# IceTTTb/NopeSAC

Measured on AMD Instinct MI355X. Metric: image-pairs/sec (480x640, K=32 hyp), higher is better.
Workload: dtype bf16; 1 GPU; configs/inference_mp3d.yaml, 32 synthetic 480x640 pairs/GPU/step, ResNet-50 + pyramids in bfloat16, head GEMMs bf16 operands with f32 accumulate / residual stream / LayerNorm / softmax, K=32 matched planes forced (m mean 32.0), nq=50; pairs_per_gpu=32, global_batch=32, K=32, parallelism=pair-sharded dp1, rccl_ranks=1, batches_in_flight_per_gpu=4, hip_graph=False, steps_per_all_gather=8, routing_entries_loaded=45, routing_entries_measured_now=0, nonfinite_outputs=0

## Files before the change

nopesac_amd/csrc/postselect.hip:

```cpp
#include "common.h"

namespace nps {

__host__ __device__ inline int work_words(int nq) { return 9 * nq + 8; }

__global__ __launch_bounds__(64) void ps_classify_kernel(const float* __restrict__ logits, int nq, float score_thr,
                                                         int* __restrict__ work) {
    const int b = blockIdx.x, lane = threadIdx.x;
    int* wk = work + (long long)b * work_words(nq);
    const float* lg = logits + (long long)b * nq * 2;
    int any = 0;
    float best_p0 = -1.f;
    int best_q = 0x7fffffff;
    for (int q = lane; q < nq; q += 64) {
        const float l0 = lg[2 * q], l1 = lg[2 * q + 1];
        const float mx = fmaxf(l0, l1);
        const float e0 = expf(l0 - mx), e1 = expf(l1 - mx);
        const float p0 = e0 / (e0 + e1), p1 = e1 / (e0 + e1);
        const int label = p1 > p0 ? 1 : 0;
        const float score = label ? p1 : p0;
        const int valid = (label == 0) && (score > score_thr);
        wk[q] = valid;
        wk[nq + q] = __float_as_int(score);
        any |= valid;
        if (p0 > best_p0) { best_p0 = p0; best_q = q; }
    }
    any = __any(any);
    if (!any) {
        for (int o = 32; o > 0; o >>= 1) {
            const float op = __shfl_xor(best_p0, o, 64);
            const int oq = __shfl_xor(best_q, o, 64);
            if (op > best_p0 || (op == best_p0 && oq < best_q)) { best_p0 = op; best_q = oq; }
        }
        if (lane == 0) {
            wk[best_q] = 1;
            wk[nq + best_q] = __float_as_int(best_p0);
        }
    }
    if (lane == 0) wk[9 * nq] = any ? 0 : 1;
}

constexpr int PS_TW = 64;
__host__ __device__ inline int ps_pad4(int nq) { return (nq + 3) & ~3; }
__host__ __device__ inline int ps_head_words(int nq) { return ((9 * nq + 3) & ~3) + 2 * ps_pad4(nq) + 4; }

__device__ __forceinline__ int mask_lane_sum(unsigned long long m) {
    return __popcll(m & 0xAAAAAAAAAAAAAAAAull) + 2 * __popcll(m & 0xCCCCCCCCCCCCCCCCull) + 4 * __popcll(m & 0xF0F0F0F0F0F0F0F0ull) +
           8 * __popcll(m & 0xFF00FF00FF00FF00ull) + 16 * __popcll(m & 0xFFFF0000FFFF0000ull) + 32 * __popcll(m & 0xFFFFFFFF00000000ull);
}

__device__ __forceinline__ int ps_writelane(int value, int lane_index, int old) {
    int saved_m0;
    asm volatile("s_mov_b32 %1, m0\n\ts_nop 4\n\ts_mov_b32 m0, %3\n\ts_nop 1\n\tv_writelane_b32 %0, %2, m0\n\ts_mov_b32 m0, %1"
                 : "+v"(old), "=&s"(saved_m0) : "s"(value), "s"(lane_index));
    return old;
}

template <int ROWS, bool X4>
__global__ __launch_bounds__(256) void ps_pixels_kernel(const float* __restrict__ prob, int nq, int h, int w, int H,
                                                        int W, float mask_thr, int src_rows, int src_cols,
                                                        int* __restrict__ work, uint8_t* __restrict__ winner, int planar, int th) {
    extern __shared__ __attribute__((aligned(16))) int sh[];
    const int nqp = ps_pad4(nq), acc_words = (9 * nq + 3) & ~3;
    int* vq = sh + acc_words;
    float* vs = reinterpret_cast<float*>(vq + nqp);
    int* nvp = vq + 2 * nqp;
    float* tile = reinterpret_cast<float*>(sh + ps_head_words(nq));
    const int b = blockIdx.z, lane = threadIdx.x & 63;
    const int wave = __builtin_amdgcn_readfirstlane(threadIdx.x >> 6);
    int* wk = work + (long long)b * work_words(nq);
    const float sch = (float)h / (float)H, scw = (float)w / (float)W;
    const int X0 = blockIdx.x * PS_TW, Y0 = blockIdx.y * th;
    const int ry0 = min((int)fmaxf(sch * (Y0 + 0.5f) - 0.5f, 0.f), h - 1);
    const int cx0 = min((int)fmaxf(scw * (X0 + 0.5f) - 0.5f, 0.f), w - 1);
    const int nrows = min(src_rows, h - ry0), ncols = min(src_cols, w - cx0);
    for (int i = threadIdx.x; i < 9 * nq; i += 256) sh[i] = 0;
    if (wave == 0) {
        int off = 0;
        for (int base = 0; base < nq; base += 64) {
            const int q = base + lane, qc = q < nq ? q : nq - 1;
            const int vl = wk[qc], sl = wk[nq + qc];
            const int v = q < nq ? vl : 0;
            const unsigned long long m = __ballot(v != 0);
            if (v) {
                const int pos = off + __popcll(m & ((1ull << lane) - 1ull));
                vq[pos] = q;
                vs[pos] = __int_as_float(sl);
            }
            off += __popcll(m);
        }
        if (lane == 0) *nvp = off;
    }
    __syncthreads();
    const int nv = *nvp, kp = ps_pad4(nv), nk4 = kp >> 2;
    if (nv == 0) return;
    if (threadIdx.x < kp - nv) { vq[nv + threadIdx.x] = vq[nv - 1]; vs[nv + threadIdx.x] = -1.f; }
    __syncthreads();
    {
        const unsigned inv = ((1u << 20) + nk4 - 1) / nk4;
        const int items = nrows * ncols * nk4;
        const long long plane = (long long)h * w;
        for (int it0 = threadIdx.x; it0 < items; it0 += 4 * 256) {
            float4 v[4];
            int dst[4];
#pragma unroll
            for (int u = 0; u < 4; ++u) {
                const int it = it0 + u * 256 < items ? it0 + u * 256 : items - 1;
                const int rc = (int)(((unsigned)it * inv) >> 20), k4 = it - rc * nk4;
                const int r = rc / ncols, c = rc - r * ncols;
                const int4 q4 = *reinterpret_cast<const int4*>(vq + 4 * k4);
                const long long pix = (long long)(ry0 + r) * w + cx0 + c;
                if (planar) {
                    const float* pb = prob + (long long)b * nq * plane + pix;
                    v[u] = make_float4(pb[q4.x * plane], pb[q4.y * plane], pb[q4.z * plane], pb[q4.w * plane]);
                } else {
                    const float* pb = prob + ((long long)b * plane + pix) * nq;
                    v[u] = make_float4(pb[q4.x], pb[q4.y], pb[q4.z], pb[q4.w]);
                }
                dst[u] = (r * src_cols + c) * kp + 4 * k4;
            }
#pragma unroll
            for (int u = 0; u < 4; ++u)
                if (it0 + u * 256 < items) *reinterpret_cast<float4*>(tile + dst[u]) = v[u];
        }
    }
    __syncthreads();
    const int X = X0 + lane;
    const float sx = fmaxf(scw * (X + 0.5f) - 0.5f, 0.f);
    const int x0 = min((int)sx, w - 1), x1 = min(x0 + 1, w - 1);
    const float lx = sx - x0, hx = 1.f - lx;
    const int c0 = min(max(x0 - cx0, 0), ncols - 1), c1 = min(max(x1 - cx0, 0), ncols - 1);
    float hy[ROWS], ly[ROWS], best[ROWS];
    int win[ROWS];
    const float *p00[ROWS], *p01[ROWS], *p10[ROWS], *p11[ROWS];
    unsigned long long inm[ROWS];
    bool in[ROWS];
#pragma unroll
    for (int r = 0; r < ROWS; ++r) {
        const int Y = X4 ? Y0 + wave * 4 + r : Y0 + r * 4 + wave;
        in[r] = X < W && Y < H;
        inm[r] = __ballot(in[r]);
        const float sy = fmaxf(sch * (Y + 0.5f) - 0.5f, 0.f);
        const int y0 = min((int)sy, h - 1), y1 = min(y0 + 1, h - 1);
        ly[r] = sy - y0; hy[r] = 1.f - ly[r];
        const int r0 = min(max(y0 - ry0, 0), nrows - 1), r1 = min(max(y1 - ry0, 0), nrows - 1);
        p00[r] = tile + (r0 * src_cols + c0) * kp; p01[r] = tile + (r0 * src_cols + c1) * kp;
        p10[r] = tile + (r1 * src_cols + c0) * kp; p11[r] = tile + (r1 * src_cols + c1) * kp;
        best[r] = -INFINITY; win[r] = -1;
    }
    int cnt_lo = 0, cnt_hi = 0;
    for (int k4 = 0; k4 < nk4; ++k4) {
        const int4 q4 = *reinterpret_cast<const int4*>(vq + 4 * k4);
        const float4 s4 = *reinterpret_cast<const float4*>(vs + 4 * k4);
        const int qv[4] = {q4.x, q4.y, q4.z, q4.w};
        const float sv[4] = {s4.x, s4.y, s4.z, s4.w};
        int np[4] = {0, 0, 0, 0};
        if constexpr (X4) {
            static_assert(!X4 || ROWS == 4, "X4 needs four rows per wave");
            float T[3][4];
#pragma unroll
            for (int sr = 0; sr < 3; ++sr) {
                const float* pa = sr == 0 ? p00[0] : (sr == 1 ? p00[2] : p10[2]);
                const float* pb = sr == 0 ? p01[0] : (sr == 1 ? p01[2] : p11[2]);
                const float4 a = *reinterpret_cast<const float4*>(pa + 4 * k4), bq = *reinterpret_cast<const float4*>(pb + 4 * k4);
                const float av[4] = {a.x, a.y, a.z, a.w}, bv[4] = {bq.x, bq.y, bq.z, bq.w};
#pragma unroll
                for (int e = 0; e < 4; ++e) T[sr][e] = hx * av[e] + lx * bv[e];
            }
#pragma unroll
            for (int r = 0; r < ROWS; ++r) {
#pragma unroll
                for (int e = 0; e < 4; ++e) {
                    const float p = hy[r] * T[r >> 1][e] + ly[r] * T[(r >> 1) + 1][e];
                    const float wgt = sv[e] * p;
                    if (wgt > best[r]) { best[r] = wgt; win[r] = qv[e]; }
                    np[e] += __popcll(__builtin_amdgcn_ballot_w64(p >= mask_thr) & inm[r]);
                }
            }
        } else
#pragma unroll
        for (int r = 0; r < ROWS; ++r) {
            const float4 a = *reinterpret_cast<const float4*>(p00[r] + 4 * k4), bq = *reinterpret_cast<const float4*>(p01[r] + 4 * k4);
            const float4 c = *reinterpret_cast<const float4*>(p10[r] + 4 * k4), d = *reinterpret_cast<const float4*>(p11[r] + 4 * k4);
            const float av[4] = {a.x, a.y, a.z, a.w}, bv[4] = {bq.x, bq.y, bq.z, bq.w}, cv[4] = {c.x, c.y, c.z, c.w}, dv[4] = {d.x, d.y, d.z, d.w};
#pragma unroll
            for (int e = 0; e < 4; ++e) {
                const float p = hy[r] * (hx * av[e] + lx * bv[e]) + ly[r] * (hx * cv[e] + lx * dv[e]);
                const float wgt = sv[e] * p;
                if (wgt > best[r]) { best[r] = wgt; win[r] = qv[e]; }
                np[e] += __popcll(__builtin_amdgcn_ballot_w64(p >= mask_thr) & inm[r]);
            }
        }
#pragma unroll
        for (int e = 0; e < 4; ++e) {
            const int k = 4 * k4 + e;
            if (k4 < 16) cnt_lo = ps_writelane(np[e], k, cnt_lo);
            else cnt_hi = ps_writelane(np[e], k - 64, cnt_hi);
        }
    }
#pragma unroll
    for (int r = 0; r < ROWS; ++r) {
        const int Y = X4 ? Y0 + wave * 4 + r : Y0 + r * 4 + wave;
        const bool ok = in[r] && win[r] >= 0;
        const bool pass = ok && best[r] > mask_thr;
        if (ok) winner[((long long)b * H + Y) * W + X] = (uint8_t)(win[r] | (pass ? 0x80 : 0));
        unsigned long long rem = __ballot(ok);
        while (rem) {
            const int w0 = __builtin_amdgcn_readlane(win[r], __ffsll((long long)rem) - 1);
            const unsigned long long m = __ballot(ok && win[r] == w0), mp = __ballot(pass && win[r] == w0);
            if (lane == 0) {
                const int cnt = __popcll(m), cp = __popcll(mp);
                atomicAdd(&sh[6 * nq + w0], cnt); atomicAdd(&sh[7 * nq + w0], X0 * cnt + mask_lane_sum(m)); atomicAdd(&sh[8 * nq + w0], Y * cnt);
                if (cp) { atomicAdd(&sh[3 * nq + w0], cp); atomicAdd(&sh[4 * nq + w0], X0 * cp + mask_lane_sum(mp)); atomicAdd(&sh[5 * nq + w0], Y * cp); }
            }
            rem &= ~m;
        }
    }
    if (lane < nv && cnt_lo) atomicAdd(&sh[2 * nq + vq[lane]], cnt_lo);
    if (lane + 64 < nv && cnt_hi) atomicAdd(&sh[2 * nq + vq[lane + 64]], cnt_hi);
    __syncthreads();
    for (int i = 2 * nq + threadIdx.x; i < 9 * nq; i += 256)
        if (sh[i]) atomicAdd(&wk[i], sh[i]);
}

__global__ __launch_bounds__(64) void ps_finalize_kernel(const float* __restrict__ params, const float* __restrict__ feat,
                                                         int nq, int D, int H, int W, float overlap_thr,
                                                         const int* __restrict__ work, int* __restrict__ n_kept,
                                                         int* __restrict__ kept_idx, float* __restrict__ planes,
                                                         float* __restrict__ feats, float* __restrict__ scores,
                                                         int* __restrict__ areas, float* __restrict__ centers,
                                                         uint8_t* __restrict__ winner, int* __restrict__ flags) {
    const int b = blockIdx.x, lane = threadIdx.x;
    const int* wk = work + (long long)b * work_words(nq);
    __shared__ int s_keep[128];
    __shared__ int s_n, s_fallback;
    const int zero_flag = wk[9 * nq];
    if (lane == 0) {
        int n = 0, fb = 0;
        double max_overlap = 0.0;
        int max_overlap_q = -1, first_valid = -1;
        for (int q = 0; q < nq; ++q) {
            if (!wk[q]) continue;
            if (first_valid < 0) first_valid = q;
            const int area = wk[3 * nq + q], orig = wk[2 * nq + q];
            if (!zero_flag) {
                if (area < 1 || orig < 1) continue;
                const double overlap = (double)area / (double)orig;
                if (overlap > max_overlap) { max_overlap = overlap; max_overlap_q = q; }
                if (overlap < (double)overlap_thr) continue;
            }
            s_keep[n++] = q;
        }
        if (n == 0) {
            s_keep[0] = max_overlap_q >= 0 ? max_overlap_q : first_valid;
            n = 1;
            fb = 1;
        }
        s_n = n;
        s_fallback = fb;
        n_kept[b] = n;
        flags[b] = (zero_flag ? 1 : 0) | (fb ? 2 : 0);
    }
    __syncthreads();
    const int n = s_n, fb = s_fallback;
    for (int i = lane; i < nq; i += 64) {
        const long long o = (long long)b * nq + i;
        if (i < n) {
            const int q = s_keep[i];
            int area, sxi, syi;
            double cx, cy;
            if (fb) {
                area = wk[6 * nq + q]; sxi = wk[7 * nq + q]; syi = wk[8 * nq + q];
                cx = ((double)sxi / W) / (double)area;
                cy = ((double)syi / H) / (double)area;
            } else {
                area = wk[3 * nq + q]; sxi = wk[4 * nq + q]; syi = wk[5 * nq + q];
                if (zero_flag && area == 0) {
                    area = 1; sxi = 0; syi = 0;
                    winner[(long long)b * H * W] = (uint8_t)(q | 0x80);
                }
                cx = ((double)sxi / W) / ((double)area + 1e-10);
                cy = ((double)syi / H) / ((double)area + 1e-10);
            }
            kept_idx[o] = q;
            areas[o] = area;
            scores[o] = __int_as_float(wk[nq + q]);
            centers[2 * o] = (float)cx;
            centers[2 * o + 1] = (float)cy;
            for (int d = 0; d < 3; ++d) planes[3 * o + d] = params[((long long)b * nq + q) * 3 + d];
        } else {
            kept_idx[o] = -1; areas[o] = 0; scores[o] = 0.f; centers[2 * o] = 0.f; centers[2 * o + 1] = 0.f;
            for (int d = 0; d < 3; ++d) planes[3 * o + d] = 0.f;
        }
    }
    for (int i = 0; i < nq; ++i) {
        const int q = i < n ? s_keep[i] : -1;
        for (int d = lane; d < D; d += 64)
            feats[((long long)b * nq + i) * D + d] = q >= 0 ? feat[((long long)b * nq + q) * D + d] : 0.f;
    }
}

}

extern "C" int nopesac_postselect_planes(const float* cls_logits, const float* mask_prob, const float* params,
                                         const float* query_feat, int B, int nq, int D, int h, int w, int H, int W,
                                         float score_thr, float mask_thr, float overlap_thr, int32_t* n_kept,
                                         int32_t* kept_idx, float* planes, float* feats, float* scores,
                                         int32_t* areas, float* centers, uint8_t* winner, int32_t* flags,
                                         int32_t* work, void* stream) {
    return nopesac_postselect_planes_ex(cls_logits, mask_prob, params, query_feat, B, nq, D, h, w, H, W, score_thr, mask_thr, overlap_thr,
                                        n_kept, kept_idx, planes, feats, scores, areas, centers, winner, flags, work, 0, stream);
}

extern "C" int nopesac_postselect_planes_ex(const float* cls_logits, const float* mask_prob, const float* params,
                                            const float* query_feat, int B, int nq, int D, int h, int w, int H, int W,
                                            float score_thr, float mask_thr, float overlap_thr, int32_t* n_kept,
                                            int32_t* kept_idx, float* planes, float* feats, float* scores,
                                            int32_t* areas, float* centers, uint8_t* winner, int32_t* flags,
                                            int32_t* work, int prob_planar, void* stream) {
    using namespace nps;
    NPS_CHECK_ARG(prob_planar == 0 || prob_planar == 1, "postselect: prob_planar must be 0 ([B,h,w,nq]) or 1 ([B,nq,h,w])");
    NPS_CHECK_ARG(cls_logits && mask_prob && params && query_feat && n_kept && kept_idx && planes && feats && scores &&
                      areas && centers && winner && flags && work, "postselect: null pointer");
    NPS_CHECK_ARG(B > 0 && nq > 0 && nq <= 128 && D > 0 && h > 0 && w > 0 && H > 0 && W > 0, "postselect: bad dims (nq<=128)");
    hipStream_t st = (hipStream_t)stream;
    hipError_t e = hipMemsetAsync(work, 0, (size_t)B * work_words(nq) * sizeof(int), st);
    if (e != hipSuccess) { set_error("postselect: memset failed: %s", hipGetErrorString(e)); return (int)e; }
    hipLaunchKernelGGL(ps_classify_kernel, dim3(B), dim3(64), 0, st, cls_logits, nq, score_thr, work);
    int th = 16, src_rows = 0;
    if (const char* e = getenv("NOPESAC_PS_TH")) { const int v = atoi(e); th = v >= 32 ? 32 : (v >= 16 ? 16 : (v >= 8 ? 8 : 4)); }
    const int src_cols = (int)(((long long)PS_TW * w + W - 1) / W) + 2;
    size_t lds = 0;
    for (;; th >>= 1) {
        src_rows = (int)(((long long)th * h + H - 1) / H) + 2;
        lds = (size_t)ps_head_words(nq) * sizeof(int) + (size_t)src_rows * src_cols * ps_pad4(nq) * sizeof(float);
        if (lds <= 64 * 1024 || th == 4) break;
    }
    NPS_CHECK_ARG(lds <= 64 * 1024, "postselect: up-sampling ratio too small for the LDS tile (%zu bytes)", lds);
    dim3 grid((W + PS_TW - 1) / PS_TW, (H + th - 1) / th, B);
    auto launch_pixels = [&](auto kern) {
        hipLaunchKernelGGL(kern, grid, dim3(256), lds, st, mask_prob, nq, h, w, H, W, mask_thr, src_rows, src_cols, work, winner,
                           prob_planar, th);
    };
    static const bool x4_off = getenv("NOPESAC_PS_X4") && atoi(getenv("NOPESAC_PS_X4")) == 0;
    if (th == 4) launch_pixels(ps_pixels_kernel<1, false>);
    else if (th == 8) launch_pixels(ps_pixels_kernel<2, false>);
    else if (th == 16 && H == 4 * h && !x4_off) launch_pixels(ps_pixels_kernel<4, true>);
    else if (th == 16) launch_pixels(ps_pixels_kernel<4, false>);
    else launch_pixels(ps_pixels_kernel<8, false>);
    hipLaunchKernelGGL(ps_finalize_kernel, dim3(B), dim3(64), 0, st, params, query_feat, nq, D, H, W, overlap_thr, work,
                       n_kept, kept_idx, planes, feats, scores, areas, centers, winner, flags);
    NPS_LAUNCH_RET();
}
```

Baseline: 4071 pairs/s.

## Prune plane candidates per tile using min/max mask-probability bounds

After loading the source tile into LDS, each block computes the per-query min and max probability over the tile with LDS atomics. It then derives a lower bound on the winning score. Queries that can never win and whose threshold outcome is uniform are dropped from the per-pixel argmax loop, and their counts are credited in bulk. This cuts the inner-loop work when few planes compete in a tile, at the cost of an extra reduction pass and barrier, and relies on the epsilon margins being safe for exactness.

```diff
diff --git a/nopesac_amd/csrc/postselect.hip b/nopesac_amd/csrc/postselect.hip
--- a/nopesac_amd/csrc/postselect.hip
+++ b/nopesac_amd/csrc/postselect.hip
@@ -41,6 +41,9 @@
 }
 
 constexpr int PS_TW = 64;
+constexpr float PS_EPS = 9.5367431640625e-07f;
+constexpr float PS_TINY = 7.888609052210118e-31f;
+constexpr unsigned PS_ONE_BITS = 0x3f800000u;
 __host__ __device__ inline int ps_pad4(int nq) { return (nq + 3) & ~3; }
 __host__ __device__ inline int ps_head_words(int nq) { return ((9 * nq + 3) & ~3) + 2 * ps_pad4(nq) + 4; }
 
@@ -59,7 +62,8 @@
 template <int ROWS, bool X4>
 __global__ __launch_bounds__(256) void ps_pixels_kernel(const float* __restrict__ prob, int nq, int h, int w, int H,
                                                         int W, float mask_thr, int src_rows, int src_cols,
-                                                        int* __restrict__ work, uint8_t* __restrict__ winner, int planar, int th) {
+                                                        int* __restrict__ work, uint8_t* __restrict__ winner, int planar, int th,
+                                                        int prune) {
     extern __shared__ __attribute__((aligned(16))) int sh[];
     const int nqp = ps_pad4(nq), acc_words = (9 * nq + 3) & ~3;
     int* vq = sh + acc_words;
@@ -92,9 +96,12 @@
         if (lane == 0) *nvp = off;
     }
     __syncthreads();
-    const int nv = *nvp, kp = ps_pad4(nv), nk4 = kp >> 2;
+    const int nv = __builtin_amdgcn_readfirstlane(*nvp), kp = ps_pad4(nv), nk4 = kp >> 2;
     if (nv == 0) return;
     if (threadIdx.x < kp - nv) { vq[nv + threadIdx.x] = vq[nv - 1]; vs[nv + threadIdx.x] = -1.f; }
+    unsigned* mnb = reinterpret_cast<unsigned*>(sh);
+    unsigned* mxb = mnb + nq;
+    if (prune && threadIdx.x < nv) mnb[threadIdx.x] = 0xffffffffu;
     __syncthreads();
     {
         const unsigned inv = ((1u << 20) + nk4 - 1) / nk4;
@@ -125,6 +132,20 @@
         }
     }
     __syncthreads();
+    if (prune) {
+        const int k = threadIdx.x % kp, g = threadIdx.x / kp, ng = 256 / kp, npos = nrows * ncols;
+        if (g < ng && k < nv) {
+            const unsigned inv = ((1u << 20) + ncols - 1) / ncols;
+            unsigned lo = 0xffffffffu, hi = 0u;
+            for (int p = g; p < npos; p += ng) {
+                const int r = (int)(((unsigned)p * inv) >> 20), c = p - r * ncols;
+                const unsigned bits = __float_as_uint(tile[(r * src_cols + c) * kp + k]);
+                lo = min(lo, bits); hi = max(hi, bits);
+            }
+            atomicMin(&mnb[k], lo); atomicMax(&mxb[k], hi);
+        }
+        __syncthreads();
+    }
     const int X = X0 + lane;
     const float sx = fmaxf(scw * (X + 0.5f) - 0.5f, 0.f);
     const int x0 = min((int)sx, w - 1), x1 = min(x0 + 1, w - 1);
@@ -149,7 +170,37 @@
         best[r] = -INFINITY; win[r] = -1;
     }
     int cnt_lo = 0, cnt_hi = 0;
+    unsigned long long cand_lo = nv >= 64 ? ~0ull : (1ull << nv) - 1ull, cand_hi = nv <= 64 ? 0ull : (nv >= 128 ? ~0ull : (1ull << (nv - 64)) - 1ull);
+    if (prune) {
+        int tot = 0;
+#pragma unroll
+        for (int r = 0; r < ROWS; ++r) tot += __popcll(inm[r]);
+        const bool thr_ok = mask_thr >= PS_TINY;
+        bool good[2], real[2];
+        float mn[2], mx[2], sc[2];
+        float lb = 0.f;
+#pragma unroll
+        for (int half = 0; half < 2; ++half) {
+            const int k = lane + 64 * half, kc = min(k, nv - 1);
+            real[half] = k < nv;
+            const unsigned hi = mxb[kc];
+            good[half] = real[half] && hi <= PS_ONE_BITS;
+            mn[half] = __uint_as_float(mnb[kc]); mx[half] = __uint_as_float(hi); sc[half] = vs[kc];
+            if (good[half]) lb = fmaxf(lb, sc[half] * (mn[half] * (1.f - PS_EPS)));
+        }
+        for (int o = 32; o > 0; o >>= 1) lb = fmaxf(lb, __shfl_xor(lb, o, 64));
+#pragma unroll
+        for (int half = 0; half < 2; ++half) {
+            const bool loses = good[half] && lb >= PS_TINY && sc[half] * (mx[half] * (1.f + PS_EPS)) < lb;
+            const bool never = good[half] && thr_ok && mx[half] * (1.f + PS_EPS) < mask_thr;
+            const bool always = good[half] && thr_ok && mn[half] * (1.f - PS_EPS) >= mask_thr;
+            const unsigned long long m = __ballot(real[half] && (!loses || !(never || always)));
+            if (half == 0) { cand_lo = m; cnt_lo = always ? tot : 0; }
+            else { cand_hi = m; cnt_hi = always ? tot : 0; }
+        }
+    }
     for (int k4 = 0; k4 < nk4; ++k4) {
+        if (!(((k4 < 16 ? cand_lo >> (4 * k4) : cand_hi >> (4 * (k4 - 16)))) & 0xFull)) continue;
         const int4 q4 = *reinterpret_cast<const int4*>(vq + 4 * k4);
         const float4 s4 = *reinterpret_cast<const float4*>(vs + 4 * k4);
         const int qv[4] = {q4.x, q4.y, q4.z, q4.w};
@@ -338,9 +389,11 @@
     }
     NPS_CHECK_ARG(lds <= 64 * 1024, "postselect: up-sampling ratio too small for the LDS tile (%zu bytes)", lds);
     dim3 grid((W + PS_TW - 1) / PS_TW, (H + th - 1) / th, B);
+    const char* pe = getenv("NOPESAC_PS_PRUNE");
+    const int prune = !(pe && atoi(pe) == 0);
     auto launch_pixels = [&](auto kern) {
         hipLaunchKernelGGL(kern, grid, dim3(256), lds, st, mask_prob, nq, h, w, H, W, mask_thr, src_rows, src_cols, work, winner,
-                           prob_planar, th);
+                           prob_planar, th, prune);
     };
     static const bool x4_off = getenv("NOPESAC_PS_X4") && atoi(getenv("NOPESAC_PS_X4")) == 0;
     if (th == 4) launch_pixels(ps_pixels_kernel<1, false>);
```

Result: no change. 4094 pairs/s, median of 6 (+0.6%).
